# nyashiki/nshogi-engine

Hardware: AMD Instinct MI355X
Metric: NN evals/sec at batch=512 (higher is better)
Workload: dtype f16m6 (f16 main term + e2m3 MX correction terms with per-32-channel E8M0 scales, f32 accumulate)

## Files before the change

nshogi-engine_amd/csrc/kernels/mfma_tile.h:

```cpp
#ifndef NSG_MFMA_TILE_H
#define NSG_MFMA_TILE_H

#include "kernels.h"

#include <atomic>
#include <type_traits>

namespace nsg {
namespace tile {

typedef float f32x4 __attribute__((ext_vector_type(4)));
typedef unsigned int u32x4 __attribute__((ext_vector_type(4)));
typedef unsigned int u32x2 __attribute__((ext_vector_type(2)));
typedef __bf16 bf16x8 __attribute__((ext_vector_type(8)));
typedef _Float16 f16x8 __attribute__((ext_vector_type(8)));

enum Mode { kConv = 0, kHeads = 1, kDense = 2 };

#ifdef NSG_COOP_SC1_STORES
constexpr bool kCoopSameXcd = false;
#else
constexpr bool kCoopSameXcd = true;
#endif
#ifdef NSG_COOP_NO_KEEP
// ... 40 lines not shown
}

template <class G, bool SHIFT = false>
__device__ __forceinline__ void zeroHalo(unsigned char* smem, int tid) {
    static_assert(G::kBoards, "board images only");
    constexpr int kBoardsN = (G::kEntries - 24) / 110;
    constexpr int kHalo = 24 + 29 * kBoardsN;
    constexpr int kPlanes = G::kLds / G::kPlane;
    const int lane = tid & 63, wave = tid >> 6;
    constexpr int kWavesN = G::kThreads / 64;
#pragma unroll
    for (int h0 = 0; h0 < kHalo; h0 += 64) {
        const int h = h0 + lane;
        int e = h;
        if (h0 + 63 >= 24) {
            const int q = h - 24, b = q / 29, r = q - b * 29;
            const int within = r < 10 ? r : (r < 19 ? (r - 9) * 10 + 9 : 81 + r);
            e = h < 24 ? h : 24 + b * 110 + within;
        }
        e = h < kHalo ? e : 0;
#pragma unroll
        for (int pl = 0; pl < (kPlanes + kWavesN - 1) / kWavesN; ++pl) {
            int plane = pl * kWavesN + wave;
            plane = plane < kPlanes ? plane : kPlanes - 1;
            if constexpr (SHIFT) {
                unsigned char* z = smem + e * 16 + (plane >> 3) * G::kBuf + (plane & 7) * G::kPlaneStride + ((plane & 7) == 7 ? 8 : 0);
                *reinterpret_cast<u32x2*>(z) = u32x2{0u, 0u};
                *reinterpret_cast<u32x2*>(z + 8) = u32x2{0u, 0u};
            } else {
                *reinterpret_cast<u32x4*>(smem + e * 16 + (plane >> 3) * G::kBuf + (plane & 7) * G::kPlaneStride) = u32x4{0u, 0u, 0u, 0u};
            }
        }
    }
}

template <int PREC>
__device__ __forceinline__ void mfmaSlab(f32x4& acc, const u32x4& w, const u32x4& a) {
    if constexpr (PREC == kFp32) {
        acc = __builtin_amdgcn_mfma_f32_16x16x4f32(__uint_as_float(w.x), __uint_as_float(a.x), acc, 0, 0, 0);
        acc = __builtin_amdgcn_mfma_f32_16x16x4f32(__uint_as_float(w.y), __uint_as_float(a.y), acc, 0, 0, 0);
        acc = __builtin_amdgcn_mfma_f32_16x16x4f32(__uint_as_float(w.z), __uint_as_float(a.z), acc, 0, 0, 0);
        acc = __builtin_amdgcn_mfma_f32_16x16x4f32(__uint_as_float(w.w), __uint_as_float(a.w), acc, 0, 0, 0);
    } else if constexpr (PREC == kFp16 || PREC == kF16x3) {
        acc = __builtin_amdgcn_mfma_f32_16x16x32_f16(__builtin_bit_cast(f16x8, w), __builtin_bit_cast(f16x8, a), acc, 0, 0, 0);
    } else {
        acc = __builtin_amdgcn_mfma_f32_16x16x32_bf16(__builtin_bit_cast(bf16x8, w), __builtin_bit_cast(bf16x8, a), acc, 0, 0, 0);
    }
}

template <int PREC>
__device__ __forceinline__ uint16_t toBits16(float v) {
    if constexpr (PREC == kFp16 || PREC == kF16x3) {
        return __builtin_bit_cast(uint16_t, (_Float16)v);
    } else {
        return __builtin_bit_cast(uint16_t, (__bf16)v);
    }
}
template <int PREC>
__device__ __forceinline__ uint32_t packPair(float lo, float hi) {
    return (uint32_t)toBits16<PREC>(lo) | ((uint32_t)toBits16<PREC>(hi) << 16);
}
template <int PREC>
__device__ __forceinline__ float unpackLo(uint32_t v) {
    if constexpr (PREC == kFp16) {
        return (float)__builtin_bit_cast(_Float16, (uint16_t)(v & 0xffffu));
    } else {
// ... 36 lines not shown
    const unsigned char* x;
    const u32x4* w;
    const float* bias;
    const unsigned char* res;
    unsigned char* y;
    float* policy;
    unsigned char* vfeat;
    int kdim;
    int cout;
    int totalRows;
    int relu;
    int valueChannels;
    int vfeatStride;
    float accScale;
    int outF16x3;
    int kSplits;
    size_t partStride;
    unsigned long long* stamps;
    int exp = 0;
};

struct ArgsTail {
    float* policy;
    unsigned char* vfeat;
    int totalRows;
    int valueChannels;
    int vfeatStride;
    int kSplits;
    size_t partStride;
    unsigned long long* stamps;
};
inline ArgsTail tailOf(const Args& a) {
    return ArgsTail{a.policy, a.vfeat, a.totalRows, a.valueChannels, a.vfeatStride, a.kSplits, a.partStride, a.stamps};
}

#ifdef NSG_DIAG_STAMPS
#define NSG_STAMP_DECL unsigned long long nsgStamp0 = 0, nsgReal0 = 0;
#define NSG_STAMP(IDX)                                                                       \
    do {                                                                                     \
        if ((IDX) == 0) {                                                                    \
            nsgStamp0 = __builtin_amdgcn_s_memtime();                                        \
            nsgReal0 = __builtin_amdgcn_s_memrealtime();                                     \
            asm volatile("s_waitcnt lgkmcnt(0)" ::: "memory");                               \
        } else if (A.stamps && threadIdx.x == 0) {                                           \
            unsigned long long* o_ = A.stamps + ((size_t)blockIdx.y * gridDim.x + blockIdx.x) * 8; \
            o_[(IDX)] = __builtin_amdgcn_s_memtime();                                        \
            if ((IDX) == 1) { o_[0] = nsgStamp0; o_[7] = nsgReal0; }                         \
            if ((IDX) == 3) o_[6] = __builtin_amdgcn_s_memrealtime();                        \
        }                                                                                    \
    } while (0)
#else
#define NSG_STAMP_DECL
#define NSG_STAMP(IDX) do { } while (0)
#endif

template <int MODE, int SIZE, int NWAVES, int NFRAG = 4, int PREC = 0>
constexpr int minWavesPerSimd() {
    return (MODE == kConv && SIZE == 1 && (NWAVES >= 3 || NFRAG <= 2) && !isMx(PREC)) ? 2 : 1;
}

template <int TAPS>
struct M8Seq {
    static constexpr int kSlabs = 3 * TAPS;
    static constexpr bool isX(int s) { return s % 3 == 2; }
    static constexpr int tap(int s) { return s / 3; }
    static constexpr int half(int s) { return s % 3; }
// ... 131 lines not shown
    static constexpr bool active(int u, int f) { return !PERM || ER::needTap(f, OS::slab(u) / 3); }
    static constexpr Tab make() {
        Tab t{};
        int n = 0;
        for (int u = 0; u < OS::kN; ++u)
            for (int f = 0; f < MF; ++f) {
                t.index[u * MF + f] = (short)(active(u, f) ? n : -1);
                if (active(u, f)) {
                    t.pos[n] = (short)u;
                    t.frag[n] = (short)f;
                    ++n;
                }
            }
        t.n = n;
        t.padded = (n + WIN - 1) / WIN * WIN;
        for (int q = n; q < kMax; ++q) { t.pos[q] = 0; t.frag[q] = -1; }
        int nx = 0;
        for (int q = 0; q < kMax; ++q) {
            t.xord[q] = (short)nx;
            if (q < n && OS::slab(t.pos[q]) % 3 == 2) ++nx;
        }
        return t;
    }
    static constexpr Tab kTab = make();
    static constexpr int kReal = kTab.n;
    static constexpr int kSteps = kTab.padded;
    static constexpr int pos(int q) { return kTab.pos[q]; }
    static constexpr int frag(int q) { return kTab.frag[q]; }
    static constexpr int index(int u, int f) { return kTab.index[u * MF + f]; }
    static constexpr int xord(int q) { return kTab.xord[q]; }
};

template <int PREC, int MODE, int SIZE, int NFRAG, int NWAVES, int RES, int MS = 1, int KS = 1, int SS = 1, int PART = 0, bool COOP = false,
          bool KEEP = false>
__device__ __forceinline__ void tileBody(const Args& A, unsigned char* smem, bool zeroLds, bool haveOwn = false) {
    static_assert(!KEEP || (COOP && SIZE == 1 && MS == 1 && KS > 1 && PREC == kF16m6), "own slice kept in LDS: cooperative K-split tiles");
    static_assert(!COOP || (isMx(PREC) && MODE == kConv && NFRAG == 4), "cooperative trunk: MX conv tiles");
    static_assert(SS == 1 || (isMx(PREC) && MODE == kConv && SIZE == 2 && MS == 1 && KS == 1 && NWAVES % SS == 0 && PART < SS),
                  "slab split: two-board MX conv tiles");
    using G = Geom<MODE, SIZE, NWAVES, (isMx(PREC) ? (KS > 1 ? 8 : 4) : 2)>;
    static_assert(KS == 1 || (isMx(PREC) && MODE == kConv && SIZE == 1 && NWAVES % KS == 0),
                  "K split: kF16m8 one-board conv tiles");
    constexpr bool kRowWG = (MS > 1 && KS > 1);
    const bool hasRes = (RES == 1) || (RES == 2 && A.res != nullptr);
    NSG_STAMP_DECL
    NSG_STAMP(0);
    constexpr bool kM8 = isMx(PREC);
    constexpr bool kM6 = (PREC == kF16m6);
    constexpr int ES = (PREC == kFp32 || PREC == kF16x3 || kM8) ? 4 : 2;
    constexpr bool kSplit = (PREC == kF16x3);
    static_assert(!kM8 || (MODE == kConv && NFRAG == 4), "kF16m8: full trunk-conv tiles only");
    static_assert(NFRAG == 1 || NFRAG == 2 || NFRAG == 4, "fragments per wave");
    static_assert(MS == 1 || (MODE == kConv && SIZE == 1 && G::kMF % MS == 0 && (KS > 1 || NWAVES % MS == 0) &&
                              (NFRAG < 4 || isMx(PREC))),
                  "row split: one-board conv tiles (small tiles, or kF16m8 full-channel tiles)");
    constexpr int kMFw = G::kMF / MS;
#ifdef NSG_NO_EDGE_ROWS
    constexpr bool kPerm = false;
#else
    constexpr bool kPerm = isMx(PREC) && MODE == kConv && NFRAG == 4 && MS == 1 && KS == 1 && (SIZE == 2 || (SIZE == 1 && kEdgeRowsOneBoard));
#endif
    using EdgeRows = std::conditional_t<SIZE == 1, EdgeRows1, EdgeRowsT<SS == 1>>;
    static_assert(!kPerm || kMFw == EdgeRows::kMF, "edge-packed rows: one table row per fragment");

    int tidOpaque = threadIdx.x;
    asm volatile("" : "+v"(tidOpaque));
    const int tid = tidOpaque;
    const int lane = tid & 63;
// ... 15 lines not shown
    const size_t lastRow = G::kBoards ? ~(size_t)0 : (size_t)(A.totalRows - 1);

    const int sli = lane >> 3, sg = lane & 7;
    size_t srcOff[G::kItems];
    int dstOff[G::kItems];
    bool itemOk[G::kItems];
#pragma unroll
    for (int k = 0; k < G::kItems; ++k) {
        const int wid = wave + k * NWAVES;
        const int m = wid * 8 + sli;
        itemOk[k] = (wid < 2 * G::kMF) && (m < G::kRows);
        size_t grow = row0 + (itemOk[k] ? m : 0);
        if (grow > lastRow) grow = lastRow;
        srcOff[k] = grow * (size_t)A.kdim * ES + sg * 16 + (size_t)kc0 * 128;
    }
    constexpr bool kTileBuf = isMx(PREC) && MODE == kConv;
    [[maybe_unused]] int srcRel[G::kItems];
    [[maybe_unused]] __amdgpu_buffer_rsrc_t xrs;
    if constexpr (kTileBuf) {
        xrs = __builtin_amdgcn_make_buffer_rsrc(const_cast<unsigned char*>(A.x) + row0 * (size_t)A.kdim * ES, 0, 0x7fffffff, 0x00027000);
#pragma unroll
        for (int k = 0; k < G::kItems; ++k) srcRel[k] = (int)(srcOff[k] - row0 * (size_t)A.kdim * ES);
    }
    auto tileLoad = [&](int k, int chunk) -> u32x4 {
        if constexpr (kTileBuf) return __builtin_bit_cast(u32x4, __builtin_amdgcn_raw_buffer_load_b128(xrs, srcRel[k], chunk * 128, COOP ? 16  : 0));
        else return *reinterpret_cast<const u32x4*>(A.x + srcOff[k] + (size_t)chunk * 128);
    };
    u32x4 st[G::kItems];
#ifdef NSG_MX_SPLIT_READ
    constexpr bool kShiftLo = (PREC == kF16m6) && MODE == kConv;
#else
    constexpr bool kShiftLo = false;
#endif
    auto stageStore = [](unsigned char* p_, const u32x4& v_) {
        if constexpr (kShiftLo) {
            *reinterpret_cast<u32x2*>(p_) = u32x2{v_.x, v_.y};
            *reinterpret_cast<u32x2*>(p_ + 8) = u32x2{v_.z, v_.w};
        } else {
            *reinterpret_cast<u32x4*>(p_) = v_;
        }
    };
    constexpr bool kResident = isMx(PREC) && KS > 1;
    constexpr int kResChunks = 8;
    constexpr int kOwnChunks = KEEP ? 2 * (NWAVES / KS) : 0;
    [[maybe_unused]] const int ownChunk0 = (int)blockIdx.y * kOwnChunks;
    u32x4 stAll[kResident ? kResChunks : 1][G::kItems];
    if constexpr (kResident) {
#pragma unroll
        for (int c = 0; c < kResChunks; ++c) {
            if (KEEP && haveOwn && c >= ownChunk0 && c < ownChunk0 + kOwnChunks) continue;
#pragma unroll
            for (int k = 0; k < G::kItems; ++k)
                stAll[c][k] = __builtin_bit_cast(u32x4, __builtin_amdgcn_raw_buffer_load_b128(
                    xrs, c < nkc ? srcRel[k] : 0x7ffffff0, c * 128, COOP ? 16  : 0));
        }
        __builtin_amdgcn_sched_barrier(0);
        NSG_STAMP(4);
    }
#pragma unroll
    for (int k = 0; k < G::kItems; ++k) {
        const int wid = wave + k * NWAVES;
        const int c = sg;
        const int mm = itemOk[k] ? wid * 8 + sli : 0;
        const int okOff = c * G::kPlaneStride + entryOfRow<G::kBoards>(mm) * 16 + ((kShiftLo && c == 7) ? 8 : 0), okMask = -(int)itemOk[k];
        dstOff[k] = (okOff & okMask) | ((G::kLds + lane * 16) & ~okMask);
    }
// ... 96 lines not shown
        auto ld4 = [&](int off_, int imm_) { return (uint32_t)__builtin_amdgcn_raw_buffer_load_b32(wrs, lane4 + imm_, off_, 0); };
        u32x4 w4[OS::kMain > 0 ? 3 : 1][NFRAG];
        u32x4 w8[OS::kX > 0 ? 2 : 1][NFRAG][kPackX ? 1 : 2];
        [[maybe_unused]] u32x2 w8b[OS::kX > 0 ? 2 : 1][NFRAG];
        [[maybe_unused]] uint32_t w8s[OS::kX > 0 ? 2 : 1];
#define NSG_M8_LOADX(SET_, OFF_, J_)                                                                            \
        _Pragma("unroll") for (int j_ = 0; j_ < NFRAG; ++j_) {                                                  \
            if ((J_) >= 0 && j_ != (J_)) continue;                                                              \
            if constexpr (kPackX) {                                                                             \
                w8[SET_][j_][0] = ld16(wc + (OFF_) + wg8, j_ * 1024);                                           \
                w8b[SET_][j_] = ld8(wc + (OFF_) + wg8 + 4096, j_ * 512);                                        \
                if ((J_) < 0 ? j_ == 0 : (J_) == 0) w8s[SET_] = ld4(wc + (OFF_) + wg8 + 4096, 2048);            \
            } else {                                                                                            \
                _Pragma("unroll") for (int h_ = 0; h_ < 2; ++h_)                                                \
                    w8[SET_][j_][kPackX ? 0 : h_] = ld16(wc + (OFF_) + wg8 + (j_ >> 1) * 4096, ((j_ & 1) * 2 + h_) * 1024); \
            }                                                                                                   \
        }
        if constexpr (OS::kMain > 0) {
#pragma unroll
            for (int o = 0; o < 2; ++o)
#pragma unroll
                for (int j = 0; j < NFRAG; ++j) w4[o][j] = ld16(wc + mainOff(OS::mainSlab(o)) + wg4, j * 1024);
        }
        if constexpr (OS::kXCyclic) { NSG_M8_LOADX(0, xOff(OS::xSlab(0)), -1) }

        if constexpr (kStage) {
        u32x4 st1[G::kItems];
#pragma unroll
        for (int k = 0; k < G::kItems; ++k) st[k] = tileLoad(k, 0);
#pragma unroll
        for (int k = 0; k < G::kItems; ++k) st1[k] = tileLoad(k, 1);
        NSG_STAMP(4);
        if constexpr (kPerm) { NSG_COMPUTE_ABASE }
        if (zeroLds) zeroHalo<G, kShiftLo>(smem, tid);
        __syncthreads();
        NSG_STAMP(5);
        NSG_STAGE_WRITE(0)
#pragma unroll
        for (int k = 0; k < G::kItems; ++k)
            stageStore(smem + (itemOk[k] ? G::kBuf : 0) + dstOff[k], st1[k]);
        __syncthreads();
        } else {
            constexpr int kChunks = kResChunks;
            if constexpr (kPerm) { NSG_COMPUTE_ABASE }
            if (zeroLds) zeroHalo<G, kShiftLo>(smem, tid);
            __syncthreads();
            NSG_STAMP(5);
#pragma unroll
            for (int c = 0; c < kChunks; ++c) {
                if (KEEP && haveOwn && c >= ownChunk0 && c < ownChunk0 + kOwnChunks) continue;
#pragma unroll
                for (int k = 0; k < G::kItems; ++k)
                    if (__builtin_expect(c < nkc, 1)) stageStore(smem + (itemOk[k] ? c * G::kBuf : 0) + dstOff[k], stAll[c][k]);
            }
            __syncthreads();
        }
        NSG_STAMP(1);

        constexpr bool kSplitRead = kShiftLo && OS::kX > 0;
        const int offB = offp8 + G::kPlaneStride + 8 * (g & 1);
        u32x4 aw[kWin][kSplitRead ? 1 : 2];
        [[maybe_unused]] u32x2 aw45[kSplitRead ? kWin : 1];
        [[maybe_unused]] uint32_t awS[kSplitRead ? kWin : 1];
#define NSG_M8_REQ(QQ, CUR, NXT)                                                                  \
        if (ST::frag((QQ) % kSteps) >= 0) {                                                       \
            const int q_ = (QQ) % kSteps;                                                         \
            const unsigned char* b_ = ((QQ) >= kSteps) ? (NXT) : (CUR);                           \
            const int s_ = OS::slab(ST::pos(q_)), f_ = ST::frag(q_);                              \
// ... 324 lines not shown
                }
                wp += slabStride;
            }
            if constexpr (kRing >= 3) {
#pragma unroll
                for (int f = 0; f < kMFw; ++f) {
                    if (dsReads) __builtin_amdgcn_sched_group_barrier(0x100, 1, 0);
                    if (wLoads && f < NFRAG) __builtin_amdgcn_sched_group_barrier(0x020, 1, 0);
                    if (kFlow && s < kLoadSlabs && f == NFRAG) __builtin_amdgcn_sched_group_barrier(0x020, kItemsPerSlab, 0);
                    if (kFlow && s == kWriteSlab && f < G::kItems)
                        __builtin_amdgcn_sched_group_barrier(0x200, 1, 0);
                    __builtin_amdgcn_sched_group_barrier(0x008, NFRAG * kMfmaPerPair, 0);
                }
            }
            __builtin_amdgcn_sched_barrier(0);
        }
        if constexpr (kWMode == 1 && (G::kTaps & 1)) {
#pragma unroll
            for (int j = 0; j < NFRAG; ++j) w[0][j] = w[2][j];
        }
        if constexpr (!kFlow) {
            NSG_STAGE_WRITE((kc + 1) & 1)
            __syncthreads();
        }
    }
    if constexpr (kFlow) __syncthreads();
    }

#undef NSG_STAGE_LOAD
#undef NSG_COMPUTE_ABASE
#undef NSG_PIN_ACC_AGPR
#undef NSG_STAGE_WRITE
    NSG_STAMP(2);

    const int nf0 = waveGroup * NFRAG;
    const int cbase = (nf0 >> 2) * 64 + g * 16 + (nf0 & 3) * 4;
    float bv[NFRAG * 4];
#pragma unroll
    for (int i = 0; i < NFRAG * 4; ++i) bv[i] = A.bias[cbase + i];

    if constexpr (MODE == kConv && NFRAG < 4) {
#pragma unroll
        for (int f = 0; f < kMFw; ++f) {
            const int m = (fBase + f) * 16 + li;
            if (m >= G::kRows) continue;
            const size_t grow = row0 + m;
            float v[NFRAG * 4];
#pragma unroll
            for (int j = 0; j < NFRAG; ++j)
#pragma unroll
                for (int r = 0; r < 4; ++r) v[j * 4 + r] = fmaf(acc[f][j][r], A.accScale, bv[j * 4 + r]);
            if constexpr (kSplit) {
                const size_t e = grow * (size_t)A.cout * 4 + (size_t)(cbase >> 5) * 128 + (cbase & 31) * 2;
                if (hasRes) {
#pragma unroll
                    for (int j = 0; j < NFRAG; ++j) {
                        const u32x2 rh = *reinterpret_cast<const u32x2*>(A.res + e + j * 8);
                        const u32x2 rl = *reinterpret_cast<const u32x2*>(A.res + e + 64 + j * 8);
#pragma unroll
                        for (int i = 0; i < 2; ++i) {
                            v[j * 4 + 2 * i] += f16BitsToF32((uint16_t)(rh[i] & 0xffffu)) + f16BitsToF32((uint16_t)(rl[i] & 0xffffu));
                            v[j * 4 + 2 * i + 1] += f16BitsToF32((uint16_t)(rh[i] >> 16)) + f16BitsToF32((uint16_t)(rl[i] >> 16));
                        }
                    }
                }
                if (A.relu) {
// ... 43 lines not shown
                            u32x2{packPair<PREC>(v[j * 4], v[j * 4 + 1]), packPair<PREC>(v[j * 4 + 2], v[j * 4 + 3])};
                    }
                }
            }
        }
        NSG_STAMP(3);
        return;
    }

#ifdef NSG_EXP_RUNTIME
    if constexpr (MODE == kConv && NFRAG == 4 && isMx(PREC)) {
        if (A.exp & 2) {
#pragma unroll
            for (int f = 0; f < kMFw; ++f)
#pragma unroll
                for (int j = 0; j < NFRAG; ++j) asm volatile("" ::"v"(acc[f][j]));
            NSG_STAMP(3);
            return;
        }
    }
#endif
    if constexpr (MODE == kConv && NFRAG == 4) {
        constexpr int kParts = KS > 1 ? KS : SS;
        constexpr int kMFe = (kMFw + kParts - 1) / kParts;
        const int fBaseE = fBase + ((KS > 1) ? (wave % KS) * kMFe : PART * kMFe);
        constexpr int kRowB = NFRAG * 16 * ES;
        constexpr int kRowS = kRowB + 16;
        constexpr int kNP = kRowB / 64;
        constexpr int kPPR = kRowB / 16;
        constexpr int kRPI = 64 / kPPR;
        constexpr int kIPF = 16 / kRPI;
        constexpr int kFragBytes = 16 * kRowS;
        constexpr int kEpiWave = G::kEpi / NWAVES / 16 * 16;
        constexpr int kRegions = (kEpiWave / kFragBytes) < 1 ? 1 : ((kEpiWave / kFragBytes) > 4 ? 4 : (kEpiWave / kFragBytes));
        static_assert(kFragBytes <= kEpiWave, "epilogue staging does not fit");
        unsigned char* ebuf = smem + wave * kEpiWave;
        const size_t rowBytes = (size_t)A.cout * ES;
        const size_t sliceOff = (size_t)waveGroup * kRowB;
        auto pieceOff = [&](int k) -> int {
            if constexpr (kSplit || kM6) return (g >> 1) * 128 + (g & 1) * 32 + (k & 1) * 16 + (k >> 1) * 64;
            else if constexpr (kM8)
                return (g >> 1) * 128 + (k < 2 ? (g & 1) * 32 + k * 16 : 64 + (k - 2) * 32 + (g & 1) * 16);
            else return g * (kRowB / 4) + k * 16;
        };
        const bool outX3 = kM8 && A.outF16x3;
        auto pieceOffX3 = [&](int k) -> int { return (g >> 1) * 128 + (g & 1) * 32 + (k & 1) * 16 + (k >> 1) * 64; };
        const int lrow = lane / kPPR;
        const int lpc = lane % kPPR;
        const unsigned laneOff = (unsigned)lrow * (unsigned)rowBytes + (unsigned)lpc * 16u;
        const size_t tileOff = (row0 + (kPerm ? (size_t)0 : (size_t)fBaseE * 16)) * rowBytes + sliceOff;
        const unsigned char* resBase = A.res + tileOff;
        unsigned char* yBase = A.y + tileOff;
        [[maybe_unused]] __amdgpu_buffer_rsrc_t resRs, yRs;
        if constexpr (COOP) {
            resRs = __builtin_amdgcn_make_buffer_rsrc(const_cast<unsigned char*>(resBase), 0, 0x7fffffff, 0x00027000);
            yRs = __builtin_amdgcn_make_buffer_rsrc(yBase, 0, 0x7fffffff, 0x00027000);
        }
        auto resLoad = [&](size_t off_) -> u32x4 {
            if constexpr (COOP) return __builtin_bit_cast(u32x4, __builtin_amdgcn_raw_buffer_load_b128(resRs, (int)off_, 0, 16));
            else return *reinterpret_cast<const u32x4*>(resBase + off_);
        };
        auto outStore = [&](size_t off_, const u32x4& v_) {
            if constexpr (COOP) __builtin_amdgcn_raw_buffer_store_b128(v_, yRs, (int)off_, 0, kCoopSameXcd ? 0 : 16);
            else *reinterpret_cast<u32x4*>(yBase + off_) = v_;
        };
        [[maybe_unused]] const unsigned permLane = (unsigned)lpc * 16u;
        const int fBasePerm = (KS > 1) ? (wave % KS) * kMFe : PART * kMFe;
        auto rowOffs = [&](int f) -> u32x4 {
            if constexpr (kPerm) return *reinterpret_cast<const u32x4*>(smem + G::kRowTabOff + ((fBasePerm + f) * 4 + lrow) * 16);
            else return u32x4{0u, 0u, 0u, 0u};
        };
        auto rowOk = [&](int f, int it, const u32x4& ro) -> bool {
            if constexpr (kPerm) return (SIZE == 2 && KS == 1 && PART * kMFe + f < EdgeRows::kMF - 1) || ro[it] != ~0u;
            else return (fBaseE + f) * 16 + it * kRPI + lrow < rowLimit;
        };
        auto rowByte = [&](int f, int it, const u32x4& ro) -> size_t {
            if constexpr (kPerm) return (size_t)(ro[it] + permLane);
            else return (size_t)(f * 16 + it * kRPI) * rowBytes + laneOff;
        };

        constexpr int kPreFrags = (RES != 1 || minWavesPerSimd<MODE, SIZE, NWAVES, NFRAG, PREC>() > 1)
                                      ? 0 : (kMFe * kIPF <= 32 ? kMFe : 32 / kIPF);
        u32x4 rpre[kPreFrags ? kPreFrags : 1][kIPF];
        if constexpr (kPreFrags > 0) {
#pragma unroll
            for (int f = 0; f < kPreFrags; ++f) {
                const u32x4 ro = rowOffs(f);
#pragma unroll
                for (int it = 0; it < kIPF; ++it) {
                    rpre[f][it] = u32x4{0u, 0u, 0u, 0u};
                    if (__builtin_expect(rowOk(f, it, ro), 1))
                        rpre[f][it] = resLoad(rowByte(f, it, ro));
                }
            }
        }

        static_assert(kRegions >= 2, "the pipelined epilogue needs two staging regions per wave");
        [[maybe_unused]] int entLi[KEEP ? kMFe : 1], entLL[KEEP ? kMFe : 1][kIPF];
        if constexpr (KEEP) {
            static_assert(kRowB == 256 && kIPF == 4, "image staging: 256-byte row slices");
            const int slice_ = waveGroup * 2 * G::kBuf;
            auto entryByte = [&](int m_) { return m_ < G::kRows ? slice_ + (34 + m_ + ((m_ * 57) >> 9)) * 16 : -1; };
            auto rowOfFrag = [&](int fg_, int r_) -> int {
                if constexpr (kPerm) {
                    int b_ = 0, y_ = 0, x_ = 0;
                    const bool ok_ = EdgeRows::square(fg_ < EdgeRows::kMF ? fg_ : 0, r_, b_, y_, x_) && fg_ < EdgeRows::kMF;
                    return ok_ ? y_ * 9 + x_ : G::kRows;
                } else {
                    return fg_ * 16 + r_;
                }
            };
#pragma unroll
            for (int f = 0; f < kMFe; ++f) {
                entLi[f] = entryByte(rowOfFrag(fBaseE + f, li));
#pragma unroll
                for (int it = 0; it < kIPF; ++it) entLL[f][it] = entryByte(rowOfFrag(fBaseE + f, it * kRPI + lrow));
            }
        }
        auto stageAt = [&](int f, int rowIsLi, int it, int piece_) -> unsigned char* {
            if constexpr (KEEP) {
                const int e_ = rowIsLi ? entLi[f] : entLL[f][it];
                return smem + (e_ < 0 ? G::kLds + lane * 16 : e_ + (piece_ >> 3) * G::kBuf + (piece_ & 7) * G::kPlaneStride);
            } else {
                return ebuf + (f % kRegions) * kFragBytes + (rowIsLi ? li : it * kRPI + lrow) * kRowS + piece_ * 16;
            }
        };
        u32x4 rpp[2][kNP];
        u32x4 tt[kIPF];
#pragma unroll
        for (int i = -1; i <= kMFe; ++i) {
            [[maybe_unused]] u32x4 roS = u32x4{0u, 0u, 0u, 0u}, roR = u32x4{0u, 0u, 0u, 0u};
            if (i >= 1) {
                const int f = i - 1;
#pragma unroll
                for (int it = 0; it < kIPF; ++it)
                    tt[it] = *reinterpret_cast<const u32x4*>(stageAt(f, 0, it, lpc));
                roS = rowOffs(f);
            }
            if (hasRes && i + 1 < kMFe) {
                const int f = i + 1;
                if (f >= kPreFrags) roR = rowOffs(f);
                const u32x4 ro = roR;
#pragma unroll
                for (int it = 0; it < kIPF; ++it) {
                    u32x4 t = u32x4{0u, 0u, 0u, 0u};
                    if (f < kPreFrags) {
                        t = rpre[f < kPreFrags ? f : 0][it];
                    } else {
                        if (__builtin_expect(rowOk(f, it, ro), 1))
                            t = resLoad(rowByte(f, it, ro));
                    }
                    *reinterpret_cast<u32x4*>(stageAt(f, 0, it, lpc)) = t;
                }
#pragma unroll
                for (int k = 0; k < kNP; ++k) {
                    const int po = (kM6 && k >= 2) ? (g >> 1) * 128 + 96 + (k - 2) * 16 : pieceOff(k);
                    rpp[f & 1][k] = *reinterpret_cast<const u32x4*>(stageAt(f, 1, 0, po / 16));
                }
            }
            if (i >= 0 && i < kMFe) {
                const int f = i;
                float v[NFRAG * 4];
#pragma unroll
                for (int j = 0; j < NFRAG; ++j)
#pragma unroll
                    for (int r = 0; r < 4; ++r) v[j * 4 + r] = fmaf(acc[f][j][r], A.accScale, bv[j * 4 + r]);
                [[maybe_unused]] unsigned char* lrowp = ebuf + (f % kRegions) * kFragBytes + li * kRowS;
                if (hasRes) {
                    const u32x4* rp = rpp[f & 1];
                    if constexpr (PREC == kFp32) {
#pragma unroll
                        for (int k = 0; k < 4; ++k)
#pragma unroll
                            for (int i = 0; i < 4; ++i) v[k * 4 + i] += __uint_as_float(rp[k][i]);
                    } else if constexpr (kSplit) {
#pragma unroll
                        for (int k = 0; k < 2; ++k)
#pragma unroll
                            for (int i = 0; i < 4; ++i) {
                                v[k * 8 + 2 * i] += f16BitsToF32((uint16_t)(rp[k][i] & 0xffffu)) +
                                                    f16BitsToF32((uint16_t)(rp[2 + k][i] & 0xffffu));
                                v[k * 8 + 2 * i + 1] += f16BitsToF32((uint16_t)(rp[k][i] >> 16)) +
                                                        f16BitsToF32((uint16_t)(rp[2 + k][i] >> 16));
                            }
                    } else if constexpr (kM6) {
                        typedef unsigned u32x6 __attribute__((ext_vector_type(6)));
                        typedef unsigned u32x16 __attribute__((ext_vector_type(16)));
                        const bool odd = (g & 1) != 0;
                        const uint32_t c0 = odd ? rp[2].w : rp[2].x, c1 = odd ? rp[3].x : rp[2].y, c2 = odd ? rp[3].y : rp[2].z;
                        const u32x6 blk = {c0, c1, c2, c0, c1, c2};
// ... 117 lines not shown
                        typedef _Float16 f16x2 __attribute__((ext_vector_type(2)));
#pragma unroll
                        for (int d = 0; d < 4; ++d) {
                            f32x2 hf[2], lf[2];
#pragma unroll
                            for (int q = 0; q < 2; ++q) {
                                const int c = 4 * d + 2 * q;
                                const f32x2 x = {__builtin_amdgcn_fmed3f(v[c], floorV, 65000.f),
                                                 __builtin_amdgcn_fmed3f(v[c + 1], floorV, 65000.f)};
                                const f16x2 h = __builtin_convertvector(x, f16x2);
                                op[c >> 3][(c & 7) >> 1] = __builtin_bit_cast(uint32_t, h);
                                const f32x2 hx = __builtin_convertvector(h, f32x2);
                                const f32x2 lx = (x - hx) * (float)(1 << kM8LoShift);
                                hf[q] = f32x2{__builtin_amdgcn_fmed3f(hx[0], -448.f, 448.f), __builtin_amdgcn_fmed3f(hx[1], -448.f, 448.f)};
                                lf[q] = f32x2{__builtin_amdgcn_fmed3f(lx[0], -448.f, 448.f), __builtin_amdgcn_fmed3f(lx[1], -448.f, 448.f)};
                            }
                            int h8 = __builtin_amdgcn_cvt_pk_fp8_f32(hf[0][0], hf[0][1], 0, false);
                            h8 = __builtin_amdgcn_cvt_pk_fp8_f32(hf[1][0], hf[1][1], h8, true);
                            int l8 = __builtin_amdgcn_cvt_pk_fp8_f32(lf[0][0], lf[0][1], 0, false);
                            l8 = __builtin_amdgcn_cvt_pk_fp8_f32(lf[1][0], lf[1][1], l8, true);
                            op[2][d] = (uint32_t)h8;
                            op[3][d] = (uint32_t)l8;
                        }
                    }
                } else {
#pragma unroll
                    for (int k = 0; k < 2; ++k)
#pragma unroll
                        for (int i = 0; i < 4; ++i) op[k][i] = packPair<PREC>(v[k * 8 + 2 * i], v[k * 8 + 2 * i + 1]);
                }
#pragma unroll
                for (int k = 0; k < kNP; ++k) {
                    if constexpr (KEEP) *reinterpret_cast<u32x4*>(stageAt(f, 1, 0, (__builtin_expect(outX3, false) ? pieceOffX3(k) : pieceOff(k)) / 16)) = op[k];
                    else *reinterpret_cast<u32x4*>(lrowp + (__builtin_expect(outX3, false) ? pieceOffX3(k) : pieceOff(k))) = op[k];
                }
            }
            if (i >= 1) {
                const int f = i - 1;
                const u32x4 ro = roS;
#pragma unroll
                for (int it = 0; it < kIPF; ++it) {
#ifdef NSG_EXP_RUNTIME
                    asm volatile("" ::"v"(tt[it]));
                    if (__builtin_expect(rowOk(f, it, ro) && !(A.exp & 1), 1))
#else
                    if (__builtin_expect(rowOk(f, it, ro), 1))
#endif
                        outStore(rowByte(f, it, ro), tt[it]);
                }
            }
        }
#ifdef NSG_DIAG_STAMPS
        asm volatile("s_waitcnt vmcnt(0)" ::: "memory");
#endif
        NSG_STAMP(3);
        return;
    }

#pragma unroll
    for (int f = 0; f < G::kMF; ++f) {
        const int m = f * 16 + li;
        const size_t grow = row0 + m;
        const bool rowOk = G::kBoards ? (m < G::kRows) : (grow <= lastRow);
        if (!rowOk) continue;
        float v[NFRAG * 4];
#pragma unroll
// ... 36 lines not shown
        }
    }
}

template <int PREC, int MODE, int SIZE, int NFRAG, int NWAVES, bool HAS_RES, int MS = 1, int KS = 1, int SS = 1>
__global__ __launch_bounds__(NWAVES * 64, (minWavesPerSimd<MODE, SIZE, NWAVES, NFRAG, PREC>())) void tileKernel(
    const unsigned char* x, const u32x4* w, const unsigned char* res, unsigned char* y, const float* bias,
    int kdim, int cout, int flags , float accScale, const ArgsTail T) {
    extern __shared__ __attribute__((aligned(16))) unsigned char smem[];
    const Args A{x, w, bias, res, y, T.policy, T.vfeat, kdim, cout, T.totalRows, flags & 1, T.valueChannels,
                 T.vfeatStride, accScale, (flags >> 1) & 1, T.kSplits, T.partStride, T.stamps, flags >> 2};
    if constexpr (SS == 1) {
        tileBody<PREC, MODE, SIZE, NFRAG, NWAVES, HAS_RES ? 1 : 0, MS, KS>(A, smem, true);
    } else {
        const int part = __builtin_amdgcn_readfirstlane((int)(threadIdx.x >> 6)) % SS;
        if (part == 0) tileBody<PREC, MODE, SIZE, NFRAG, NWAVES, HAS_RES ? 1 : 0, MS, KS, SS, 0>(A, smem, true);
        else if (part == 1) tileBody<PREC, MODE, SIZE, NFRAG, NWAVES, HAS_RES ? 1 : 0, MS, KS, SS, 1>(A, smem, true);
        else if constexpr (SS > 2) {
            if (part == 2) tileBody<PREC, MODE, SIZE, NFRAG, NWAVES, HAS_RES ? 1 : 0, MS, KS, SS, 2>(A, smem, true);
            else tileBody<PREC, MODE, SIZE, NFRAG, NWAVES, HAS_RES ? 1 : 0, MS, KS, SS, 3>(A, smem, true);
        }
    }
}

template <int PREC, int SIZE, int NFRAG, int NWAVES>
__global__ __launch_bounds__(NWAVES * 64, (minWavesPerSimd<kConv, SIZE, NWAVES, NFRAG, PREC>())) void trunkKernel(
    const Args* __restrict__ layers, int nLayers, int skewTicks) {
    extern __shared__ __attribute__((aligned(16))) unsigned char smem[];
    if (skewTicks > 0) {
        const unsigned long long t0 = __builtin_amdgcn_s_memrealtime();
        const unsigned long long wait = (unsigned long long)skewTicks * ((blockIdx.x >> 3) & 7);
        while (__builtin_amdgcn_s_memrealtime() - t0 < wait) __builtin_amdgcn_s_sleep(16);
    }
    for (int l = 0; l < nLayers; ++l) {
        const Args A = layers[l];
        if (A.res) tileBody<PREC, kConv, SIZE, NFRAG, NWAVES, 1>(A, smem, true);
        else tileBody<PREC, kConv, SIZE, NFRAG, NWAVES, 0>(A, smem, true);
        __syncthreads();
    }
}

template <int PREC, int NFRAG, int NWAVES, int MS, int KS>
__global__ __launch_bounds__(NWAVES * 64, 1) void coopTrunkKernel(const Args* __restrict__ layers, int nLayers, int boards,
                                                                  unsigned* flags, unsigned flagBase, int* status, int faultBoard) {
    extern __shared__ __attribute__((aligned(16))) unsigned char smem[];
    using G = Geom<kConv, 1, NWAVES, 8>;
    if ((int)blockIdx.x >= boards) return;
    const int members = (int)(gridDim.y * gridDim.z), me = (int)(blockIdx.z * gridDim.y + blockIdx.y);
    if ((int)blockIdx.x == faultBoard && me == 1) return;
    unsigned xcc = 0;
    if constexpr (kCoopSameXcd) {
        asm volatile("s_getreg_b32 %0, hwreg(HW_REG_XCC_ID, 0, 4)" : "=s"(xcc));
        if (faultBoard == -2 && me == 1) xcc ^= 1u;
    }
    int* gaveUp = reinterpret_cast<int*>(smem + G::kLdsAlloc);
    unsigned* mine = flags + (size_t)blockIdx.x * members;
    if (threadIdx.x == 0) *gaveUp = 0;
    for (int l = 0; l < nLayers; ++l) {
        const Args A = layers[l];
        asm volatile("" ::"s"(A.x), "s"(A.w), "s"(A.res), "s"(A.y), "s"(A.bias), "s"(A.kdim), "s"(A.cout), "s"(A.relu), "s"(A.accScale),
                     "s"(A.outF16x3));
        if (l > 0) {
            if ((int)threadIdx.x < members && (int)threadIdx.x != me) {
                int spins = 0;
                unsigned seen;
                while (((seen = __hip_atomic_load(mine + threadIdx.x, __ATOMIC_RELAXED, __HIP_MEMORY_SCOPE_AGENT)) & 0xffffffu) < flagBase + (unsigned)l) {
                    if ((++spins & 255) == 0 &&
                        (spins > (1 << 21) || __hip_atomic_load(status, __ATOMIC_RELAXED, __HIP_MEMORY_SCOPE_SYSTEM) != 0)) {
                        __hip_atomic_store(status, 1, __ATOMIC_RELAXED, __HIP_MEMORY_SCOPE_SYSTEM);
                        *gaveUp = 1;
                        seen = xcc << 24;
// ... 162 lines not shown
```

Measured before the change: 202,400.

## Stage trunk epilogue in interior LDS slots and clear halo once per launch

For the f16m6 trunk kernel, the epilogue staging buffers are remapped onto interior (non-halo) entries of the per-wave LDS image. A constexpr check verifies that staging never touches halo slots, so the halo zeroing and its barrier run only on the first layer instead of every layer. The next layer's Args are prefetched through constant-address-space scalar loads during the current layer's epilogue and pinned in SGPRs, hiding the per-layer argument fetch. The costs are more complex addressing in the epilogue and a dependency on the LDS layout invariant holding.

After: 204,200 (median of 6 runs). About the same (+0.9%).

```diff
diff --git a/nshogi-engine_amd/csrc/kernels/mfma_tile.h b/nshogi-engine_amd/csrc/kernels/mfma_tile.h
--- a/nshogi-engine_amd/csrc/kernels/mfma_tile.h
+++ b/nshogi-engine_amd/csrc/kernels/mfma_tile.h
@@ -96,6 +96,43 @@
             }
         }
     }
+}
+
+template <class G>
+struct EpiImageMap {
+    static constexpr int kBoardsN = (G::kEntries - 24) / 110;
+    static constexpr int kRegions = 2 * kBoardsN;
+    static constexpr int kHalfEntries = 40;
+    static constexpr int regionEntry(int r) { return 34 + (r >> 1) * 110 + (r & 1) * 20; }
+    static constexpr int rowEntry(int row) { return (row >> 3) * 10 + (row & 7); }
+    static constexpr int byteOf(int wave, int r, int row, int piece) {
+        return wave * G::kBuf + (piece & 7) * G::kPlaneStride + (regionEntry(r) + (piece >> 3) * kHalfEntries + rowEntry(row)) * 16;
+    }
+    static constexpr bool isHalo(int e) {
+        if (e < 24) return true;
+        const int q = (e - 24) % 110;
+        return q < 10 || q >= 100 || q % 10 == 9;
+    }
+    static constexpr bool offHalo(int nwaves) {
+        for (int w = 0; w < nwaves; ++w)
+            for (int r = 0; r < kRegions; ++r)
+                for (int row = 0; row < 16; ++row)
+                    for (int p = 0; p < 16; ++p) {
+                        const int b = byteOf(w, r, row, p);
+                        const int within = b % G::kBuf, plane = within / G::kPlaneStride, off = within % G::kPlaneStride;
+                        if (b / G::kBuf >= G::kLds / G::kBuf || b / G::kBuf != w || plane != (p & 7) || off % 16 != 0) return false;
+                        if (off / 16 >= G::kEntries || isHalo(off / 16)) return false;
+                    }
+        return true;
+    }
+};
+template <int PREC>
+constexpr bool epiOffHalo() {
+#ifdef NSG_MX_SPLIT_READ
+    return false;
+#else
+    return PREC == kF16m6;
+#endif
 }
 
 template <int PREC>
@@ -198,6 +235,40 @@
 };
 inline ArgsTail tailOf(const Args& a) {
     return ArgsTail{a.policy, a.vfeat, a.totalRows, a.valueChannels, a.vfeatStride, a.kSplits, a.partStride, a.stamps};
+}
+
+template <class T>
+__device__ __forceinline__ T constLoad(const T* p) {
+    return *(const __attribute__((address_space(4))) T*)p;
+}
+__device__ __forceinline__ void loadArgsConst(Args& o, const Args* p) {
+    o.x = constLoad(&p->x); o.w = constLoad(&p->w); o.bias = constLoad(&p->bias); o.res = constLoad(&p->res);
+    o.y = constLoad(&p->y); o.policy = constLoad(&p->policy); o.vfeat = constLoad(&p->vfeat);
+    o.kdim = constLoad(&p->kdim); o.cout = constLoad(&p->cout); o.totalRows = constLoad(&p->totalRows);
+    o.relu = constLoad(&p->relu); o.valueChannels = constLoad(&p->valueChannels); o.vfeatStride = constLoad(&p->vfeatStride);
+    o.accScale = constLoad(&p->accScale); o.outF16x3 = constLoad(&p->outF16x3); o.kSplits = constLoad(&p->kSplits);
+    o.partStride = constLoad(&p->partStride); o.stamps = constLoad(&p->stamps); o.exp = constLoad(&p->exp);
+}
+__device__ __forceinline__ void pinArgs(Args& o) {
+    asm volatile("" : "+s"(o.x), "+s"(o.w), "+s"(o.bias), "+s"(o.res), "+s"(o.y), "+s"(o.kdim), "+s"(o.cout), "+s"(o.relu),
+                      "+s"(o.accScale), "+s"(o.outF16x3), "+s"(o.stamps), "+s"(o.exp));
+}
+template <class T>
+__device__ __forceinline__ T firstLane(T v) {
+    if constexpr (sizeof(T) == 4) {
+        return __builtin_bit_cast(T, __builtin_amdgcn_readfirstlane(__builtin_bit_cast(int, v)));
+    } else {
+        static_assert(sizeof(T) == 8, "dwords and pointers");
+        const unsigned long long u = __builtin_bit_cast(unsigned long long, v);
+        const unsigned lo = (unsigned)__builtin_amdgcn_readfirstlane((int)(unsigned)u);
+        const unsigned hi = (unsigned)__builtin_amdgcn_readfirstlane((int)(unsigned)(u >> 32));
+        return __builtin_bit_cast(T, (unsigned long long)lo | ((unsigned long long)hi << 32));
+    }
+}
+__device__ __forceinline__ void firstLaneArgs(Args& o, const Args& a) {
+    o.x = firstLane(a.x); o.w = firstLane(a.w); o.bias = firstLane(a.bias); o.res = firstLane(a.res); o.y = firstLane(a.y);
+    o.kdim = firstLane(a.kdim); o.cout = firstLane(a.cout); o.relu = firstLane(a.relu); o.accScale = firstLane(a.accScale);
+    o.outF16x3 = firstLane(a.outF16x3); o.stamps = firstLane(a.stamps); o.exp = firstLane(a.exp);
 }
 
 #ifdef NSG_DIAG_STAMPS
@@ -395,8 +466,9 @@
 };
 
 template <int PREC, int MODE, int SIZE, int NFRAG, int NWAVES, int RES, int MS = 1, int KS = 1, int SS = 1, int PART = 0, bool COOP = false,
-          bool KEEP = false>
-__device__ __forceinline__ void tileBody(const Args& A, unsigned char* smem, bool zeroLds, bool haveOwn = false) {
+          bool KEEP = false, bool TRUNK = false>
+__device__ __forceinline__ void tileBody(const Args& A, unsigned char* smem, bool zeroLds, bool haveOwn = false,
+                                         [[maybe_unused]] const Args* nextArgs = nullptr, [[maybe_unused]] Args* nextOut = nullptr) {
     static_assert(!KEEP || (COOP && SIZE == 1 && MS == 1 && KS > 1 && PREC == kF16m6), "own slice kept in LDS: cooperative K-split tiles");
     static_assert(!COOP || (isMx(PREC) && MODE == kConv && NFRAG == 4), "cooperative trunk: MX conv tiles");
     static_assert(SS == 1 || (isMx(PREC) && MODE == kConv && SIZE == 2 && MS == 1 && KS == 1 && NWAVES % SS == 0 && PART < SS),
@@ -478,6 +550,8 @@
 #else
     constexpr bool kShiftLo = false;
 #endif
+    constexpr bool kEpiOffHalo = TRUNK && epiOffHalo<PREC>() && MODE == kConv && NFRAG == 4 && MS == 1 && KS == 1 && SS == 1 && !KEEP;
+    static_assert(!kEpiOffHalo || !kShiftLo, "interior staging: pieces on their slots");
     auto stageStore = [](unsigned char* p_, const u32x4& v_) {
         if constexpr (kShiftLo) {
             *reinterpret_cast<u32x2*>(p_) = u32x2{v_.x, v_.y};
@@ -640,8 +714,15 @@
         for (int k = 0; k < G::kItems; ++k) st1[k] = tileLoad(k, 1);
         NSG_STAMP(4);
         if constexpr (kPerm) { NSG_COMPUTE_ABASE }
-        if (zeroLds) zeroHalo<G, kShiftLo>(smem, tid);
-        __syncthreads();
+        if constexpr (kEpiOffHalo) {
+            if (zeroLds) {
+                zeroHalo<G, kShiftLo>(smem, tid);
+                __syncthreads();
+            }
+        } else {
+            if (zeroLds) zeroHalo<G, kShiftLo>(smem, tid);
+            __syncthreads();
+        }
         NSG_STAMP(5);
         NSG_STAGE_WRITE(0)
 #pragma unroll
@@ -1032,6 +1113,7 @@
 #undef NSG_PIN_ACC_AGPR
 #undef NSG_STAGE_WRITE
     NSG_STAMP(2);
+    if constexpr (TRUNK) loadArgsConst(*nextOut, nextArgs);
 
     const int nf0 = waveGroup * NFRAG;
     const int cbase = (nf0 >> 2) * 64 + g * 16 + (nf0 & 3) * 4;
@@ -1141,8 +1223,14 @@
         constexpr int kIPF = 16 / kRPI;
         constexpr int kFragBytes = 16 * kRowS;
         constexpr int kEpiWave = G::kEpi / NWAVES / 16 * 16;
-        constexpr int kRegions = (kEpiWave / kFragBytes) < 1 ? 1 : ((kEpiWave / kFragBytes) > 4 ? 4 : (kEpiWave / kFragBytes));
+        using EM = EpiImageMap<G>;
+        constexpr int kRegions = kEpiOffHalo ? EM::kRegions
+                                             : ((kEpiWave / kFragBytes) < 1 ? 1 : ((kEpiWave / kFragBytes) > 4 ? 4 : (kEpiWave / kFragBytes)));
         static_assert(kFragBytes <= kEpiWave, "epilogue staging does not fit");
+        if constexpr (kEpiOffHalo) {
+            static_assert(kRowB == 256 && kRPI == 4 && NWAVES * G::kBuf <= G::kLds, "interior staging: 256-byte row slices, a buffer per wave");
+            static_assert(EM::offHalo(NWAVES), "epilogue staging must not overwrite a halo entry: the halo is cleared once per launch");
+        }
         unsigned char* ebuf = smem + wave * kEpiWave;
         const size_t rowBytes = (size_t)A.cout * ES;
         const size_t sliceOff = (size_t)waveGroup * kRowB;
@@ -1156,6 +1244,12 @@
         auto pieceOffX3 = [&](int k) -> int { return (g >> 1) * 128 + (g & 1) * 32 + (k & 1) * 16 + (k >> 1) * 64; };
         const int lrow = lane / kPPR;
         const int lpc = lane % kPPR;
+        [[maybe_unused]] const int emLL = wave * G::kBuf + (lpc & 7) * G::kPlaneStride + ((lpc >> 3) * EM::kHalfEntries + lrow) * 16;
+        [[maybe_unused]] const int emMFr = wave * G::kBuf + ((g >> 1) * EM::kHalfEntries + EM::rowEntry(li)) * 16;
+        [[maybe_unused]] const int emMF = emMFr + (g & 1) * 2 * G::kPlaneStride;
+        [[maybe_unused]] auto stageMf = [&](int f, bool withG1, int cp_) -> unsigned char* {
+            return smem + (withG1 ? emMF : emMFr) + EM::regionEntry(f % kRegions) * 16 + cp_ * G::kPlaneStride;
+        };
         const unsigned laneOff = (unsigned)lrow * (unsigned)rowBytes + (unsigned)lpc * 16u;
         const size_t tileOff = (row0 + (kPerm ? (size_t)0 : (size_t)fBaseE * 16)) * rowBytes + sliceOff;
         const unsigned char* resBase = A.res + tileOff;
@@ -1205,6 +1299,7 @@
         }
 
         static_assert(kRegions >= 2, "the pipelined epilogue needs two staging regions per wave");
+        if constexpr (TRUNK) pinArgs(*nextOut);
         [[maybe_unused]] int entLi[KEEP ? kMFe : 1], entLL[KEEP ? kMFe : 1][kIPF];
         if constexpr (KEEP) {
             static_assert(kRowB == 256 && kIPF == 4, "image staging: 256-byte row slices");
@@ -1230,6 +1325,8 @@
             if constexpr (KEEP) {
                 const int e_ = rowIsLi ? entLi[f] : entLL[f][it];
                 return smem + (e_ < 0 ? G::kLds + lane * 16 : e_ + (piece_ >> 3) * G::kBuf + (piece_ & 7) * G::kPlaneStride);
+            } else if constexpr (kEpiOffHalo) {
+                return smem + emLL + (EM::regionEntry(f % kRegions) + EM::rowEntry(it * kRPI)) * 16;
             } else {
                 return ebuf + (f % kRegions) * kFragBytes + (rowIsLi ? li : it * kRPI + lrow) * kRowS + piece_ * 16;
             }
@@ -1263,8 +1360,9 @@
                 }
 #pragma unroll
                 for (int k = 0; k < kNP; ++k) {
-                    const int po = (kM6 && k >= 2) ? (g >> 1) * 128 + 96 + (k - 2) * 16 : pieceOff(k);
-                    rpp[f & 1][k] = *reinterpret_cast<const u32x4*>(stageAt(f, 1, 0, po / 16));
+                    [[maybe_unused]] const int po = (kM6 && k >= 2) ? (g >> 1) * 128 + 96 + (k - 2) * 16 : pieceOff(k);
+                    if constexpr (kEpiOffHalo) rpp[f & 1][k] = *reinterpret_cast<const u32x4*>(k >= 2 ? stageMf(f, false, 6 + (k - 2)) : stageMf(f, true, k));
+                    else rpp[f & 1][k] = *reinterpret_cast<const u32x4*>(stageAt(f, 1, 0, po / 16));
                 }
             }
             if (i >= 0 && i < kMFe) {
@@ -1448,6 +1546,7 @@
 #pragma unroll
                 for (int k = 0; k < kNP; ++k) {
                     if constexpr (KEEP) *reinterpret_cast<u32x4*>(stageAt(f, 1, 0, (__builtin_expect(outX3, false) ? pieceOffX3(k) : pieceOff(k)) / 16)) = op[k];
+                    else if constexpr (kEpiOffHalo) *reinterpret_cast<u32x4*>(stageMf(f, true, (k & 1) + (k >> 1) * 4)) = op[k];
                     else *reinterpret_cast<u32x4*>(lrowp + (__builtin_expect(outX3, false) ? pieceOffX3(k) : pieceOff(k))) = op[k];
                 }
             }
@@ -1550,11 +1649,17 @@
         const unsigned long long wait = (unsigned long long)skewTicks * ((blockIdx.x >> 3) & 7);
         while (__builtin_amdgcn_s_memrealtime() - t0 < wait) __builtin_amdgcn_s_sleep(16);
     }
+    constexpr bool kZeroOnce = epiOffHalo<PREC>() && NFRAG == 4;
+    Args A;
+    loadArgsConst(A, layers);
     for (int l = 0; l < nLayers; ++l) {
-        const Args A = layers[l];
-        if (A.res) tileBody<PREC, kConv, SIZE, NFRAG, NWAVES, 1>(A, smem, true);
-        else tileBody<PREC, kConv, SIZE, NFRAG, NWAVES, 0>(A, smem, true);
+        const Args* nextArgs = layers + (l + 1 < nLayers ? l + 1 : l);
+        Args An;
+        const bool zero = !kZeroOnce || l == 0;
+        if (A.res) tileBody<PREC, kConv, SIZE, NFRAG, NWAVES, 1, 1, 1, 1, 0, false, false, true>(A, smem, zero, false, nextArgs, &An);
+        else tileBody<PREC, kConv, SIZE, NFRAG, NWAVES, 0, 1, 1, 1, 0, false, false, true>(A, smem, zero, false, nextArgs, &An);
         __syncthreads();
+        firstLaneArgs(A, An);
     }
 }
 
```
